# XchaoWu/ScaNeRF-Scalable-Bundle-Adjusting-Neural-Radiance-Fields-for-Large-Scale-Scene-Rendering

Hardware: NVIDIA B200
Metric: train rays/s (fwd+bwd) (higher is better)
Workload: dtype f32

## Files before the change

include/scanerf_b200.h:

```cpp
#ifndef SCANERF_B200_H
#define SCANERF_B200_H

#ifdef __cplusplus
extern "C" {
#endif

const char* snrf_last_error(void);
int snrf_version(void);
int snrf_device_sm_count(void);
int snrf_l2_fetch_granularity(int bytes);

int snrf_hash_fwd(const float* points, const float* table, const int* res, const float* corner,
                  const float* size, void* out, unsigned* idx_out, int B, int L, int T, int out_bf16,
                  void* stream);
int snrf_hash_bwd(const float* points, const float* grad_in, const float* table, const int* res,
                  const float* corner, const float* size, float* grad_points, float* grad_table,
                  int B, int L, int T, int aggregate_levels, void* stream);
void snrf_hash_set_levels_per_block(int lpb);

int snrf_field_encode_fwd(const float* rays_o, const float* rays_d, const float* z_vals, const float* points,
                          const float* box_min, const float* box_size, int mode, const float* table, const int* res,
                          float* out_lm, float* jac_lm, const unsigned char* ray_valid, int split, int N, int S, int L, int T,
                          void* stream);
int snrf_field_encode_bwd(const float* rays_o, const float* rays_d, const float* z_vals, const float* points,
// ... 63 lines not shown
                           int s_sigma, int s_tint, int s_diffuse, int s_specular,
                           const float* z_vals, const float* dists, const float* rays_d, const unsigned char* ray_valid,
                           int R, int S, int infinity, int inf_start, float* weights, float* trans, float* out,
                           float ert_eps, unsigned char* sample_live, void* stream);
int snrf_composite_bwd_ert(const float* sigma, const float* tint, const float* diffuse, const float* specular,
                           int s_sigma, int s_tint, int s_diffuse, int s_specular,
                           const float* z_vals, const float* dists, const float* rays_d, const float* trans,
                           const float* g_out, const float* g_weights, const unsigned char* ray_valid, int R, int S, int infinity,
                           int inf_start, float* g_sigma, float* g_tint, float* g_diffuse, float* g_specular,
                           int gs_sigma, int gs_tint, int gs_diffuse, int gs_specular,
                           float* grad_rays_d, const unsigned char* sample_live, void* stream);
int snrf_decoder_bwd_ert(const float* feats, const float* mask32, const float* rays_d, const float* const* params,
                         const float* grad_heads, float* grad_feats, float* grad_rays_d, float* const* grad_params,
                         int N, int S, int level_major, const unsigned char* ray_valid, const float* heads_fwd,
                         const unsigned char* sample_live, void* stream);
int snrf_field_encode_bwd_ert(const float* rays_o, const float* rays_d, const float* z_vals, const float* points,
                              const float* box_min, const float* box_size, int mode, const int* res, const float* grad_lm,
                              const float* jac_lm, float* grad_rays_o, float* grad_rays_d, float* grad_points, float* grad_table,
                              const unsigned char* ray_valid, int split, int N, int S, int L, int T,
                              const unsigned char* sample_live, void* stream);
int snrf_field_encode_bwd_adam_ert(const float* rays_o, const float* rays_d, const float* z_vals, const float* points,
                                   const float* box_min, const float* box_size, int mode, const int* res, const float* grad_lm,
                                   const float* jac_lm, float* grad_rays_o, float* grad_rays_d, float* grad_points,
                                   float* table, float* exp_avg, float* exp_avg_sq, float lr, float beta1, float beta2, float eps,
                                   int step, float* grad_scratch, long long scratch_entries, int small_levels, float* cpts_scratch,
                                   const unsigned char* ray_valid, int split, int N, int S, int L, int T,
                                   const unsigned char* sample_live, void* stream);

int snrf_joint_loss(const float* row, const unsigned char* valid_f, const unsigned char* valid_b, const float* gt,
                    float l2_weight, int R, float* loss, float* g_row, float* pred_color, int* counts_scratch, void* stream);

int snrf_umma_selftest(const float* X, const float* W, const float* G, float* Y, float* DX, float* DW,
                       float* DWo, float* YS, void* stream);

int snrf_decoder_fwd(const float* feats, const float* mask32, const float* rays_d, const float* const* params,
                     float* heads, int N, int S, int level_major, const unsigned char* ray_valid, void* stream);

void snrf_decoder_set_precision(int split);
void snrf_decoder_set_inflight(int n);
void snrf_decoder_set_fwd_fold(int on);
void snrf_decoder_set_bwd_merged(int on);
int snrf_decoder_bwd(const float* feats, const float* mask32, const float* rays_d, const float* const* params,
                     const float* grad_heads, float* grad_feats, float* grad_rays_d, float* const* grad_params,
                     int N, int S, int level_major, const unsigned char* ray_valid, const float* heads_fwd, void* stream);

int snrf_view_cost(const float* rays_o, const float* rays_d, const float* pts, const float* ks, const float* rts,
                   float* costs, int n_cam, int B, int height, int width, void* stream);
int snrf_proj2nei_fwd(const float* pts, const float* ks, const float* rts, const int* nei_views,
                      const unsigned char* nei_valid, float* nei_origin, float* nei_direction, float* grid, int B, int K,
                      void* stream);
int snrf_proj2nei_bwd(const float* pts, const float* ks, const float* rts, const int* nei_views,
                      const unsigned char* nei_valid, const float* dL_dgrid, float* grad_pts, float* grad_rts, int B, int K,
                      int n_cam, void* stream);
int snrf_grid_sample_fwd(const unsigned char* src, const float* grid, float* out, unsigned char* mask, int n_img, int B,
                         int height, int width, void* stream);
int snrf_grid_sample_bwd(const unsigned char* src, const float* grid, const float* grad_in, float* grad_grid, int n_img,
                         int B, int height, int width, void* stream);
int snrf_gauss_sample_fwd(const unsigned char* src, const float* grid, float* out, unsigned char* mask, int n_img, int B,
                          int height, int width, float sigma, float max_dis, void* stream);
int snrf_gauss_sample_bwd(const unsigned char* src, const float* grid, const float* grad_in, float* grad_grid, int n_img,
                          int B, int height, int width, float sigma, float max_dis, void* stream);
int snrf_nei_sample_fwd(const unsigned char* images, const unsigned char* occlusion, const float* grid, const int* nei_views,
                        const unsigned char* nei_valid, float* color, unsigned char* valid_out, int B, int K, int height,
                        int width, void* stream);
int snrf_nei_sample_bwd(const unsigned char* images, const float* grid, const int* nei_views, const unsigned char* nei_valid,
                        const float* grad_color, float* grad_grid, int B, int K, int height, int width, void* stream);
// ... 76 lines not shown
```

scanerf-scalable-bundle-adjusting-neural-radiance-fields-for-large-scale-scene-rendering_b200/csrc/decoder.cu:

```cuda
#include "decoder_core.cuh"

using namespace dec;

namespace {

constexpr bool kWgradDzLo = false;

template <bool SPLIT>
__global__ void __launch_bounds__(kThreadsDec, 1)
decoder_fwd_kernel(const float* __restrict__ feats, const float* __restrict__ mask32, const float* __restrict__ rays_d,
                   DecoderParams p, float* __restrict__ out, int N, int S, int num_tiles, long long level_stride,
                   const unsigned char* __restrict__ ray_valid)
{
    extern __shared__ __align__(1024) unsigned char smem_raw[];
    unsigned char* smem = (unsigned char*)(((uintptr_t)smem_raw + 1023) & ~(uintptr_t)1023);
    __shared__ uint64_t bars[2];
    __shared__ uint32_t tmem_slot;
    const int tid = threadIdx.x, warp = tid >> 5;

    stage_all_weights<SPLIT>(smem, p, mask32, tid, kThreadsDec);
    if (warp == 0) umma::tmem_alloc<512>(&tmem_slot);
    if (tid == 0) { umma::mbar_init(&bars[0], 1); umma::mbar_init(&bars[1], 1); umma::mbar_fence_init(); }
    umma::fence_async_smem();
    umma::tc_fence_before();
// ... 523 lines not shown
#pragma unroll
        for (int off = 16; off > 0; off >>= 1) {
            t2 += __shfl_xor_sync(0xffffffffu, t2, off);
            t4 += __shfl_xor_sync(0xffffffffu, t4, off);
        }
        if (lane == 0 && !first) {
            atomicAdd(gp.b2 + (j < 8 ? 8 * cg + j : 32 + 8 * cg + (j - 8)), t2 * ginv);
            atomicAdd(gp.b4 + 16 * cg + j, t4 * ginv);
        }
    }
    if (cg == 0) {
#pragma unroll
        for (int j = 0; j < 10; ++j) {
            float t = acc_small[j];
#pragma unroll
            for (int off = 16; off > 0; off >>= 1) t += __shfl_xor_sync(0xffffffffu, t, off);
            if (lane == 0 && !first) {
                float* dst = j == 0 ? gp.bs : (j < 4 ? gp.bd + (j - 1) : (j < 7 ? gp.bt + (j - 4) : gp.b5 + (j - 7)));
                atomicAdd(dst, t * ginv);
            }
        }
    }
    umma::tc_fence_before();
    __syncthreads();
    if (warp == 0) umma::tmem_free<512>(tmem);
}

namespace fold {
constexpr int oW1 = 0, oW32 = 8192, oW32l = 16384, oW3b = 24576, oW4 = 32768, oW4l = 40960, oWh2 = 49152, oWh2l = 51200,
              oW5 = 53248, oW5l = 55296, weights_end = 57344;
constexpr int oB1 = 0, oB32 = 64, oB4 = 128, nB = 192;
constexpr int off_bias = weights_end, off_mask = off_bias + nB * 4;
constexpr int off_tiles = ((off_mask + 128 + 1023) / 1024) * 1024;
constexpr int kTiles = 9;
constexpr int smem_bytes = off_tiles + kTiles * kTile + 1024;
constexpr int cDa = 0, cDb = 64, cSH = 128, gW1 = 144, gG = 192, gW3b = 256, gW4 = 272, gGhT = 336, gW5T = 352;
}

template <bool SPLIT>
__global__ void __launch_bounds__(kThreadsDec, 1)
decoder_bwd_fold_kernel(const float* __restrict__ feats, const float* __restrict__ mask32, const float* __restrict__ rays_d,
                        DecoderParams p, const float* __restrict__ grad_heads, float* __restrict__ grad_feats,
                        float* __restrict__ grad_rays_d, DecoderGrads gp, int N, int S, int num_tiles, long long level_stride,
                        const unsigned char* __restrict__ ray_valid, const unsigned* __restrict__ gmax_bits,
                        const float* __restrict__ heads_fwd, const unsigned char* __restrict__ sample_live)
{
    using namespace fold;
    extern __shared__ __align__(1024) unsigned char smem_raw[];
    unsigned char* smem = (unsigned char*)(((uintptr_t)smem_raw + 1023) & ~(uintptr_t)1023);
    unsigned char* base = smem + off_tiles;
    unsigned char *tA0 = base, *tLOb = base + kTile, *ta1 = base + 2 * kTile, *tg1 = base + 3 * kTile, *ta3 = base + 4 * kTile,
                  *tg3 = base + 5 * kTile, *ta4 = base + 6 * kTile, *tg4 = base + 7 * kTile, *tLOa = base + 8 * kTile;
    unsigned char* Tdz = tLOb;
    __shared__ uint64_t bar;
    __shared__ uint64_t bar_tail;
    __shared__ uint32_t tmem_slot;
    const int tid = threadIdx.x, warp = tid >> 5, lane = tid & 31;
    uint32_t tail_phase = 0, phase = 0;
    bool tail_pending = false;
    float gscale = 1.0f, ginv = 1.0f;
    if (kOpBf16 == 0 && gmax_bits != nullptr) {
        const int e = (int)((*gmax_bits >> 23) & 0xffu);
        if (e > 0 && e < 255) {
            int se = 253 - e;
            se = se < 1 ? 1 : (se > 253 ? 253 : se);
            gscale = __uint_as_float((uint32_t)se << 23);
            ginv = __uint_as_float((uint32_t)(254 - se) << 23);
        }
    }

    for (int i = tid; i < weights_end / 16; i += kThreadsDec) reinterpret_cast<uint4*>(smem)[i] = make_uint4(0u, 0u, 0u, 0u);
    float* s32 = reinterpret_cast<float*>(base);
    float* sh2 = s32 + 64 * 64;
    float* sW2 = sh2 + 8 * 64;
    float* sW3a = sW2 + 64 * 65;
    float* sWh = sW3a + 64 * 33;
    float* sb2 = sWh + 8 * 33;
    auto load_factors = [&]() {
        for (int i = tid; i < 64 * 64; i += kThreadsDec) sW2[(i >> 6) * 65 + (i & 63)] = w_at(p.W2, i >> 6, i & 63, 64, 64, p.flat);
        for (int i = tid; i < 64 * 32; i += kThreadsDec) sW3a[(i >> 5) * 33 + (i & 31)] = w_at(p.W3, i >> 5, i & 31, 64, 48, p.flat);
        for (int i = tid; i < 7 * 32; i += kThreadsDec) sWh[(i >> 5) * 33 + (i & 31)] = wh_at(p, i >> 5, i & 31);
        for (int i = tid; i < 64; i += kThreadsDec) sb2[i] = p.b2[i];
    };
    float* bias = reinterpret_cast<float*>(smem + off_bias);
    float* maskv = reinterpret_cast<float*>(smem + off_mask);
    load_factors();
// ... 21 lines not shown
            for (int k = 0; k < 32; ++k) v += sW3a[o * 33 + k] * sb2[32 + k];
        } else v = p.b4[i - 128];
        bias[i] = v;
    }
    for (int i = tid; i < 32; i += kThreadsDec) maskv[i] = mask32 ? mask32[i] : 1.0f;
    __syncthreads();
    stage_weight<SPLIT>(smem + oW1, smem + oW1, 0, p.W1, 64, 32, p.flat, tid, kThreadsDec);
    stage_weight<SPLIT>(smem + oW4, smem + oW4l, 0, p.W4, 64, 64, p.flat, tid, kThreadsDec);
    stage_weight<SPLIT>(smem + oW5, smem + oW5l, 0, p.W5, 3, 64, p.flat, tid, kThreadsDec);
    stage_weight<SPLIT>(smem + oW32, smem + oW32l, 0, s32, 64, 64, 0, tid, kThreadsDec);
    stage_weight<SPLIT>(smem + oWh2, smem + oWh2l, 0, sh2, 7, 64, 0, tid, kThreadsDec);
    for (int t = tid; t < 64 * 2; t += kThreadsDec) {
        const int r = t >> 1, c = t & 1;
        float hi[8], lo[8];
#pragma unroll
        for (int j = 0; j < 8; ++j) {
            const float w = w_at(p.W3, r, 32 + 8 * c + j, 64, 48, p.flat);
            hi[j] = w;
            lo[j] = w - op_round(w);
        }
        op_tile_store8(smem + oW3b, r, c, hi);
        if (SPLIT) op_tile_store8(smem + oW3b, r, 4 + c, lo);
    }
    if (warp == 0) umma::tmem_alloc<512>(&tmem_slot);
    if (tid == 0) { umma::mbar_init(&bar, 1); umma::mbar_init(&bar_tail, 1); umma::mbar_fence_init(); }
    umma::fence_async_smem();
    umma::tc_fence_before();
    __syncthreads();
    umma::tc_fence_after();

    const int row = 32 * (warp & 3) + lane, cg = warp >> 2;
    const uint32_t tmem = tmem_slot, lane_addr = (uint32_t)(32 * (warp & 3)) << 16;
    const uint32_t aA0 = umma::smem_u32(tA0), aa1 = umma::smem_u32(ta1), ag1 = umma::smem_u32(tg1), aa3 = umma::smem_u32(ta3),
                   ag3 = umma::smem_u32(tg3), aa4 = umma::smem_u32(ta4), ag4 = umma::smem_u32(tg4), aLOa = umma::smem_u32(tLOa),
                   aLOb = umma::smem_u32(tLOb), adz = aLOb;
    const uint32_t aW1 = umma::smem_u32(smem + oW1), aW32 = umma::smem_u32(smem + oW32), aW32l = umma::smem_u32(smem + oW32l),
                   aW3b = umma::smem_u32(smem + oW3b), aW4 = umma::smem_u32(smem + oW4), aW4l = umma::smem_u32(smem + oW4l),
                   aWh2 = umma::smem_u32(smem + oWh2), aWh2l = umma::smem_u32(smem + oWh2l), aW5 = umma::smem_u32(smem + oW5),
                   aW5l = umma::smem_u32(smem + oW5l);
    constexpr uint32_t idf64 = umma::idesc_f16(128, 64, 0, 0, kOpBf16, kOpBf16);
    constexpr uint32_t idg64 = umma::idesc_f16(128, 64, 0, 1, kOpBf16, kOpBf16), idg32 = umma::idesc_f16(128, 32, 0, 1, kOpBf16, kOpBf16),
                       idg16 = umma::idesc_f16(128, 16, 0, 1, kOpBf16, kOpBf16);
    constexpr uint32_t idw64 = umma::idesc_f16(64, 64, 1, 1, kOpBf16, kOpBf16), idw48 = umma::idesc_f16(64, 48, 1, 1, kOpBf16, kOpBf16),
                       idw16 = umma::idesc_f16(64, 16, 1, 1, kOpBf16, kOpBf16);
    auto dgrad = [&](int col, uint32_t dz_tile, int dz_k, uint32_t dzlo_tile, int dzlo_k, uint32_t w_hi, uint32_t w_lo, int nk,
                     uint32_t idesc, bool acc) {
        for (int k = 0; k < nk; ++k)
            umma::mma_bf16(tmem + col, umma::desc_kmajor(dz_tile, dz_k + k), umma::desc_mnmajor(w_hi, k), idesc, acc || k > 0);
        if (SPLIT) {
            for (int k = 0; k < nk; ++k)
                umma::mma_bf16(tmem + col, umma::desc_kmajor(dz_tile, dz_k + k), umma::desc_mnmajor(w_lo, k), idesc, 1);
            for (int k = 0; k < nk; ++k)
                umma::mma_bf16(tmem + col, umma::desc_kmajor(dzlo_tile, dzlo_k + k), umma::desc_mnmajor(w_hi, k), idesc, 1);
        }
    };
    auto wgrad = [&](int col, uint32_t a_tile, uint32_t b_tile_plus_off, uint32_t idesc, bool init) {
        for (int k = 0; k < 8; ++k)
            umma::mma_bf16(tmem + col, umma::desc_mnmajor(a_tile, k), umma::desc_mnmajor(b_tile_plus_off, k), idesc, (!init) || k > 0);
    };
    auto sync_operands = [&]() {
        umma::fence_async_smem();
        umma::tc_fence_before();
        __syncthreads();
        umma::tc_fence_after();
    };
    auto wait_mma = [&]() {
        umma::mbar_wait(&bar, phase);
        phase ^= 1u;
        umma::tc_fence_after();
    };
    float v[16];
    float acc_b4[16], acc_small[10];
#pragma unroll
    for (int j = 0; j < 16; ++j) acc_b4[j] = 0.0f;
#pragma unroll
    for (int j = 0; j < 10; ++j) acc_small[j] = 0.0f;
    auto gauss_epilogue = [&](int col, int boff, unsigned char* Ta, unsigned char* Tlo, unsigned char* Tg) {
        float g[16];
        umma::tmem_ld16(tmem + col + lane_addr + 16 * cg, v);
        umma::tc_wait_ld();
#pragma unroll
        for (int j = 0; j < 16; ++j) {
            const float z = v[j] + bias[boff + 16 * cg + j];
            const float a = gauss_act(z);
            v[j] = a;
            g[j] = -100.0f * z * a;
        }
#pragma unroll
        for (int q = 0; q < 2; ++q) {
            store8_act<SPLIT>(Ta, 2 * cg + q, Tlo, 2 * cg + q, row, v + 8 * q);
            umma::tile_store8_f16(Tg, row, 2 * cg + q, g + 8 * q);
        }
    };
    auto mul_inplace = [&](int col, unsigned char* Tg, unsigned char* Tlo) {
        umma::tmem_ld16(tmem + col + lane_addr + 16 * cg, v);
        umma::tc_wait_ld();
#pragma unroll
        for (int q = 0; q < 2; ++q) {
            const uint4 w4 = *reinterpret_cast<const uint4*>(Tg + umma::tile_chunk_off(row, 2 * cg + q));
            const uint32_t w[4] = {w4.x, w4.y, w4.z, w4.w};
            float o[8];
#pragma unroll
            for (int e = 0; e < 4; ++e) {
                const __half2 h2 = *reinterpret_cast<const __half2*>(&w[e]);
                o[2 * e] = v[8 * q + 2 * e] * __low2float(h2);
                o[2 * e + 1] = v[8 * q + 2 * e + 1] * __high2float(h2);
            }
            store8_act<SPLIT>(Tg, 2 * cg + q, Tlo, 2 * cg + q, row, o);
        }
    };
    const bool lead_warp = umma::warp_uniform() == 4;
    bool first = true;
    for (int tile = blockIdx.x; tile < num_tiles; tile += gridDim.x) {
        const int n = tile * kRows + row;
        const bool live = n < N && (ray_valid == nullptr || ray_valid[n / S] != 0) && (sample_live == nullptr || sample_live[n] != 0);
        if ((ray_valid != nullptr || sample_live != nullptr) && !__syncthreads_or(live)) continue;
        if (cg == 0 && live) {
            prefetch_l2(grad_heads + (size_t)n * 10);
            prefetch_l2(grad_heads + (size_t)n * 10 + 8);
            prefetch_l2(heads_fwd + (size_t)n * 10);
            prefetch_l2(heads_fwd + (size_t)n * 10 + 8);
        }
        {
            const long long nn = (long long)(tile + gridDim.x) * kRows + row;
            if (nn < N) {
                if (level_stride == 0) prefetch_l2(feats + (size_t)nn * 32 + 8 * cg);
                else {
#pragma unroll
                    for (int l = 0; l < 4; ++l) if ((row & 3) == 0) prefetch_l2(reinterpret_cast<const float2*>(feats) + nn + (size_t)(4 * cg + l) * level_stride);
                }
            }
        }
        f3 d = mk3(0.f, 0.f, 1.f);
        float dn = 1.0f;
        {
            float x[8];
#pragma unroll
            for (int j = 0; j < 8; ++j) x[j] = 0.0f;
            if (live) {
                if (level_stride == 0) {
#pragma unroll
                    for (int q = 0; q < 2; ++q) {
                        const float4 a = __ldg(reinterpret_cast<const float4*>(feats + (size_t)n * 32 + 8 * cg + 4 * q));
                        x[4 * q] = a.x; x[4 * q + 1] = a.y; x[4 * q + 2] = a.z; x[4 * q + 3] = a.w;
                    }
                } else {
                    const float2* f2 = reinterpret_cast<const float2*>(feats) + n;
#pragma unroll
                    for (int l = 0; l < 4; ++l) {
                        const float2 a = __ldg(f2 + (size_t)(4 * cg + l) * level_stride);
                        x[2 * l] = a.x; x[2 * l + 1] = a.y;
                    }
                }
                if (cg >= 2) d = ld3(rays_d + 3 * (size_t)(n / S));
#pragma unroll
                for (int j = 0; j < 8; ++j) x[j] *= maskv[8 * cg + j];
            }
            if (tail_pending) {
                umma::mbar_wait(&bar_tail, tail_phase);
                umma::tc_fence_after();
                tail_phase ^= 1u;
                tail_pending = false;
            }
            store8_act<SPLIT>(tA0, cg, tLOb, cg, row, x);
        }
        sync_operands();
        if (lead_warp && umma::elect_one()) {
            fwd_gemm<SPLIT>(tmem + cDa, aA0, 0, aLOb, 0, aW1, 0, aW1, 2, 2, idf64, false);
            umma::mma_commit(&bar);
        }
        if (cg >= 2) {
            float sh[16];
#pragma unroll
            for (int j = 0; j < 16; ++j) sh[j] = 0.0f;
            if (live) {
                dn = sqrtf(d.x * d.x + d.y * d.y + d.z * d.z);
                const float inv = 1.0f / (dn + 1e-8f);
                sh16(d.x * inv, d.y * inv, d.z * inv, sh);
            }
            store8_act<SPLIT>(tA0, 4 + (cg - 2), tA0, 6 + (cg - 2), row, sh + 8 * (cg - 2));
            if (!SPLIT) umma::tile_zero8(tA0, row, 6 + (cg - 2));
        }
        wait_mma();
        gauss_epilogue(cDa, oB1, ta1, tLOa, tg1);
        sync_operands();
        if (lead_warp && umma::elect_one()) {
            fwd_gemm<SPLIT>(tmem + cDb, aa1, 0, aLOa, 0, aW32, 0, aW32l, 0, 4, idf64, false);
            fwd_gemm<SPLIT>(tmem + cDb, aA0, 2, aA0, 3, aW3b, 0, aW3b, 2, 1, idf64, true);
            umma::mma_commit(&bar);
        }
        if (cg == 0) {
            float dzh[16], dzs[16], gh[10], hv[10];
            if (live) {
                const float2* gsrc = reinterpret_cast<const float2*>(grad_heads + (size_t)n * 10);
                const float2* hsrc = reinterpret_cast<const float2*>(heads_fwd + (size_t)n * 10);
#pragma unroll
                for (int j = 0; j < 5; ++j) {
                    const float2 t = __ldg(gsrc + j), h = __ldg(hsrc + j);
                    gh[2 * j] = t.x * gscale; gh[2 * j + 1] = t.y * gscale;
                    hv[2 * j] = h.x; hv[2 * j + 1] = h.y;
                }
            } else {
#pragma unroll
                for (int j = 0; j < 10; ++j) { gh[j] = 0.0f; hv[j] = 0.0f; }
            }
#pragma unroll
            for (int j = 0; j < 16; ++j) { dzh[j] = 0.0f; dzs[j] = 0.0f; }
            dzh[0] = gh[0] * (hv[0] > 20.0f ? 1.0f : -expm1f(-hv[0]));
#pragma unroll
            for (int j = 0; j < 3; ++j) {
                dzh[1 + j] = gh[4 + j] * hv[4 + j] * (1.0f - hv[4 + j]);
                dzh[4 + j] = gh[1 + j] * hv[1 + j] * (1.0f - hv[1 + j]);
                dzs[j] = gh[7 + j] * hv[7 + j] * (1.0f - hv[7 + j]);
            }
            store8_act<SPLIT>(Tdz, 0, Tdz, 4, row, dzh);
            store8_act<SPLIT>(Tdz, 1, Tdz, 5, row, dzh + 8);
            store8_act<SPLIT>(Tdz, 2, Tdz, 6, row, dzs);
            store8_act<SPLIT>(Tdz, 3, Tdz, 7, row, dzs + 8);
#pragma unroll
            for (int j = 0; j < 10; ++j) acc_small[j] += j < 7 ? dzh[j] : dzs[j - 7];
        }
        wait_mma();
        gauss_epilogue(cDb, oB32, ta3, tLOa, tg3);
        sync_operands();
        if (lead_warp && umma::elect_one()) {
            fwd_gemm<SPLIT>(tmem + cDa, aa3, 0, aLOa, 0, aW4, 0, aW4l, 0, 4, idf64, false);
            dgrad(cDb, adz, 1, adz, 3, aW5, aW5l, 1, idg64, false);
            umma::mma_commit(&bar);
            wgrad(gGhT, aa1, adz, idw16, first);
        }
        wait_mma();
        {
            float z4[16];
            umma::tmem_ld16(tmem + cDa + lane_addr + 16 * cg, z4);
            umma::tmem_ld16(tmem + cDb + lane_addr + 16 * cg, v);
            umma::tc_wait_ld();
#pragma unroll
            for (int j = 0; j < 16; ++j) {
                const float z = z4[j] + bias[oB4 + 16 * cg + j];
                const float a = gauss_act(z);
                z4[j] = a;
                v[j] *= -100.0f * z * a;
                acc_b4[j] += v[j];
            }
#pragma unroll
            for (int q = 0; q < 2; ++q) {
                umma::tile_store8_f16(ta4, row, 2 * cg + q, z4 + 8 * q);
                store8_act<SPLIT>(tg4, 2 * cg + q, tLOa, 2 * cg + q, row, v + 8 * q);
            }
        }
        sync_operands();
        if (lead_warp && umma::elect_one()) {
            dgrad(cDa, ag4, 0, aLOa, 0, aW4, aW4l, 4, idg64, false);
            umma::mma_commit(&bar);
            wgrad(gW4, ag4, aa3, idw64, first);
            wgrad(gW5T, aa4, adz + 32, idw16, first);
        }
        wait_mma();
        mul_inplace(cDa, tg3, tLOa);
        sync_operands();
        if (lead_warp && umma::elect_one()) {
            dgrad(cDb, ag3, 0, aLOa, 0, aW32, aW32l, 4, idg64, false);
            dgrad(cDb, adz, 0, adz, 2, aWh2, aWh2l, 1, idg64, true);
            dgrad(cSH, ag3, 0, aLOa, 0, aW3b, aW3b + 64, 4, idg16, false);
            umma::mma_commit(&bar);
            wgrad(gG, ag3, aa1, idw64, first);
            wgrad(gW3b, ag3, aA0 + 64, idw16, first);
        }
        wait_mma();
        mul_inplace(cDb, tg1, tLOa);
        sync_operands();
        if (lead_warp && umma::elect_one()) {
            dgrad(cDa, ag1, 0, aLOa, 0, aW1, aW1 + 64, 4, idg32, false);
            umma::mma_commit(&bar);
            wgrad(gW1, ag1, aA0, idw48, first);
            umma::mma_commit(&bar_tail);
        }
        if (grad_rays_d != nullptr && cg == 3) {
            float dsh[16];
            umma::tmem_ld16(tmem + cSH + lane_addr, dsh);
            umma::tc_wait_ld();
            float gx = 0.f, gy = 0.f, gz = 0.f;
            if (live) {
                const float inv = 1.0f / (dn + 1e-8f);
                const float x = d.x * inv, y = d.y * inv, z = d.z * inv;
                const float xx = x * x, yy = y * y, zz = z * z, xy = x * y, yz = y * z, xz = x * z;
                const float C1 = 0.4886025119029199f, C2a = 1.0925484305920792f, C2c = 0.31539156525252005f,
                            C2e = 0.5462742152960396f, C3a = 0.5900435899266435f, C3b = 2.890611442640554f,
                            C3c = 0.4570457994644658f, C3d = 0.3731763325901154f, C3e = 1.445305721320277f;
                float vx = 0.f, vy = 0.f, vz = 0.f;
                vy += dsh[1] * C1; vz += dsh[2] * C1; vx += dsh[3] * C1;
                vx += dsh[4] * C2a * y; vy += dsh[4] * C2a * x;
                vy += dsh[5] * -C2a * z; vz += dsh[5] * -C2a * y;
                vx += dsh[6] * C2c * -2.f * x; vy += dsh[6] * C2c * -2.f * y; vz += dsh[6] * C2c * 4.f * z;
                vx += dsh[7] * -C2a * z; vz += dsh[7] * -C2a * x;
                vx += dsh[8] * C2e * 2.f * x; vy += dsh[8] * C2e * -2.f * y;
                vx += dsh[9] * -C3a * 6.f * xy; vy += dsh[9] * -C3a * (3.f * xx - 3.f * yy);
                vx += dsh[10] * C3b * yz; vy += dsh[10] * C3b * xz; vz += dsh[10] * C3b * xy;
                vx += dsh[11] * -C3c * -2.f * xy; vy += dsh[11] * -C3c * (4.f * zz - xx - 3.f * yy); vz += dsh[11] * -C3c * 8.f * yz;
                vx += dsh[12] * C3d * -6.f * xz; vy += dsh[12] * C3d * -6.f * yz; vz += dsh[12] * C3d * (6.f * zz - 3.f * xx - 3.f * yy);
                vx += dsh[13] * -C3c * (4.f * zz - 3.f * xx - yy); vy += dsh[13] * -C3c * -2.f * xy; vz += dsh[13] * -C3c * 8.f * xz;
                vx += dsh[14] * C3e * 2.f * xz; vy += dsh[14] * C3e * -2.f * yz; vz += dsh[14] * C3e * (xx - yy);
                vx += dsh[15] * -C3a * (3.f * xx - 3.f * yy); vy += dsh[15] * -C3a * -6.f * xy;
                const float ddv = d.x * vx + d.y * vy + d.z * vz;
                const float k2 = dn > 0.f ? ddv * inv * inv / dn : 0.f;
                gx = (vx * inv - d.x * k2) * ginv; gy = (vy * inv - d.y * k2) * ginv; gz = (vz * inv - d.z * k2) * ginv;
// ... 301 lines not shown
```

scanerf-scalable-bundle-adjusting-neural-radiance-fields-for-large-scale-scene-rendering_b200/csrc/umma.cuh:

```cuda
#pragma once
#include <cuda_bf16.h>
#include <cuda_fp16.h>
#include <stdint.h>

namespace umma {

__device__ __forceinline__ uint32_t smem_u32(const void* p) { return (uint32_t)__cvta_generic_to_shared(p); }

__device__ __forceinline__ void mbar_init(uint64_t* bar, uint32_t count)
{
    asm volatile("mbarrier.init.shared::cta.b64 [%0], %1;" ::"r"(smem_u32(bar)), "r"(count));
}
__device__ __forceinline__ void mbar_fence_init() { asm volatile("fence.mbarrier_init.release.cluster;" ::: "memory"); }
__device__ __forceinline__ void mbar_wait(uint64_t* bar, uint32_t parity)
{
    asm volatile(
        "{\n"
        ".reg .pred P1;\n"
        "LAB_WAIT:\n"
        "mbarrier.try_wait.parity.shared::cta.b64 P1, [%0], %1;\n"
        "@P1 bra DONE;\n"
        "bra LAB_WAIT;\n"
        "DONE:\n"
        "}\n" ::"r"(smem_u32(bar)), "r"(parity)
// ... 34 lines not shown

__host__ __device__ constexpr uint32_t idesc_bf16(int M, int N, int a_mn_major, int b_mn_major)
{
    return (1u << 4) | (1u << 7) | (1u << 10) | ((uint32_t)a_mn_major << 15) | ((uint32_t)b_mn_major << 16) |
           ((uint32_t)(N >> 3) << 17) | ((uint32_t)(M >> 4) << 24);
}
__host__ __device__ constexpr uint32_t idesc_f16(int M, int N, int a_mn_major, int b_mn_major, int a_bf16, int b_bf16)
{
    return (1u << 4) | ((uint32_t)a_bf16 << 7) | ((uint32_t)b_bf16 << 10) | ((uint32_t)a_mn_major << 15) | ((uint32_t)b_mn_major << 16) |
           ((uint32_t)(N >> 3) << 17) | ((uint32_t)(M >> 4) << 24);
}

__device__ __forceinline__ bool elect_one()
{
    uint32_t pred;
    asm volatile(
        "{\n"
        ".reg .pred P1;\n"
        "elect.sync _|P1, 0xFFFFFFFF;\n"
        "selp.b32 %0, 1, 0, P1;\n"
        "}\n"
        : "=r"(pred));
    return pred != 0;
}
__device__ __forceinline__ int warp_uniform() { return __shfl_sync(0xffffffffu, (int)(threadIdx.x >> 5), 0); }
__device__ __forceinline__ void mma_bf16(uint32_t tmem_d, uint64_t adesc, uint64_t bdesc, uint32_t idesc, uint32_t accumulate)
{
    asm volatile(
        "{\n"
        ".reg .pred p;\n"
        "setp.ne.b32 p, %4, 0;\n"
        "tcgen05.mma.cta_group::1.kind::f16 [%0], %1, %2, %3, p;\n"
        "}\n" ::"r"(tmem_d), "l"(adesc), "l"(bdesc), "r"(idesc), "r"(accumulate)
        : "memory");
}
__device__ __forceinline__ void mma_commit(uint64_t* bar)
{
    asm volatile("tcgen05.commit.cta_group::1.mbarrier::arrive::one.shared::cluster.b64 [%0];" ::"r"(smem_u32(bar)) : "memory");
}

__device__ __forceinline__ void tmem_ld32(uint32_t taddr, float* v)
{
    uint32_t* r = reinterpret_cast<uint32_t*>(v);
    asm volatile(
        "tcgen05.ld.sync.aligned.32x32b.x32.b32 "
        "{%0, %1, %2, %3, %4, %5, %6, %7, %8, %9, %10, %11, %12, %13, %14, %15, "
        "%16, %17, %18, %19, %20, %21, %22, %23, %24, %25, %26, %27, %28, %29, %30, %31}, [%32];"
        : "=r"(r[0]), "=r"(r[1]), "=r"(r[2]), "=r"(r[3]), "=r"(r[4]), "=r"(r[5]), "=r"(r[6]), "=r"(r[7]), "=r"(r[8]),
          "=r"(r[9]), "=r"(r[10]), "=r"(r[11]), "=r"(r[12]), "=r"(r[13]), "=r"(r[14]), "=r"(r[15]), "=r"(r[16]),
          "=r"(r[17]), "=r"(r[18]), "=r"(r[19]), "=r"(r[20]), "=r"(r[21]), "=r"(r[22]), "=r"(r[23]), "=r"(r[24]),
          "=r"(r[25]), "=r"(r[26]), "=r"(r[27]), "=r"(r[28]), "=r"(r[29]), "=r"(r[30]), "=r"(r[31])
        : "r"(taddr)
        : "memory");
}
__device__ __forceinline__ void tmem_ld16(uint32_t taddr, float* v)
{
    uint32_t* r = reinterpret_cast<uint32_t*>(v);
    asm volatile(
        "tcgen05.ld.sync.aligned.32x32b.x16.b32 "
        "{%0, %1, %2, %3, %4, %5, %6, %7, %8, %9, %10, %11, %12, %13, %14, %15}, [%16];"
        : "=r"(r[0]), "=r"(r[1]), "=r"(r[2]), "=r"(r[3]), "=r"(r[4]), "=r"(r[5]), "=r"(r[6]), "=r"(r[7]), "=r"(r[8]),
          "=r"(r[9]), "=r"(r[10]), "=r"(r[11]), "=r"(r[12]), "=r"(r[13]), "=r"(r[14]), "=r"(r[15])
        : "r"(taddr)
        : "memory");
}
__device__ __forceinline__ void tmem_ld8(uint32_t taddr, float* v)
{
    uint32_t* r = reinterpret_cast<uint32_t*>(v);
    asm volatile("tcgen05.ld.sync.aligned.32x32b.x8.b32 {%0, %1, %2, %3, %4, %5, %6, %7}, [%8];"
                 : "=r"(r[0]), "=r"(r[1]), "=r"(r[2]), "=r"(r[3]), "=r"(r[4]), "=r"(r[5]), "=r"(r[6]), "=r"(r[7])
                 : "r"(taddr)
                 : "memory");
}
__device__ __forceinline__ uint32_t tmem_addr(uint32_t base, int lane, int col) { return base + ((uint32_t)lane << 16) + (uint32_t)col; }

__device__ __forceinline__ uint32_t tile_chunk_off(int row, int chunk) { return (uint32_t)row * 128u + (uint32_t)((chunk ^ (row & 7)) << 4); }

__device__ __forceinline__ uint32_t pack_bf16(float a, float b)
{
    __nv_bfloat162 h = __floats2bfloat162_rn(a, b);
    return *reinterpret_cast<uint32_t*>(&h);
}
__device__ __forceinline__ uint32_t pack_f16(float a, float b)
{
    uint32_t r;
    asm("cvt.rn.satfinite.f16x2.f32 %0, %1, %2;" : "=r"(r) : "f"(b), "f"(a));
    return r;
}
__device__ __forceinline__ void tile_store8(unsigned char* tile, int row, int chunk, const float* v)
{
    uint4 q;
    q.x = pack_bf16(v[0], v[1]); q.y = pack_bf16(v[2], v[3]); q.z = pack_bf16(v[4], v[5]); q.w = pack_bf16(v[6], v[7]);
    *reinterpret_cast<uint4*>(tile + tile_chunk_off(row, chunk)) = q;
}
__device__ __forceinline__ void tile_store8_f16(unsigned char* tile, int row, int chunk, const float* v)
{
    uint4 q;
    q.x = pack_f16(v[0], v[1]); q.y = pack_f16(v[2], v[3]); q.z = pack_f16(v[4], v[5]); q.w = pack_f16(v[6], v[7]);
    *reinterpret_cast<uint4*>(tile + tile_chunk_off(row, chunk)) = q;
}
__device__ __forceinline__ void tile_zero8(unsigned char* tile, int row, int chunk)
{
    *reinterpret_cast<uint4*>(tile + tile_chunk_off(row, chunk)) = make_uint4(0u, 0u, 0u, 0u);
}

}
```

scanerf-scalable-bundle-adjusting-neural-radiance-fields-for-large-scale-scene-rendering_b200/csrc/umma_selftest.cu:

```cuda
#include "common.cuh"
#include "umma.cuh"

namespace {

__global__ void __launch_bounds__(128, 1)
umma_selftest_kernel(const float* __restrict__ X, const float* __restrict__ W, const float* __restrict__ G,
                     float* __restrict__ Y, float* __restrict__ DX, float* __restrict__ DW,
                     float* __restrict__ DWo, float* __restrict__ YS)
{
    extern __shared__ __align__(1024) unsigned char smem_raw[];
    unsigned char* smem = (unsigned char*)(((uintptr_t)smem_raw + 1023) & ~(uintptr_t)1023);
    unsigned char* tX = smem;
    unsigned char* tG = smem + 16384;
    unsigned char* tW = smem + 32768;
    __shared__ uint64_t bar;
    __shared__ uint32_t tmem_base_slot;

    const int tid = threadIdx.x, warp = tid >> 5;
    for (int c = 0; c < 8; ++c) {
        umma::tile_store8(tX, tid, c, X + tid * 64 + c * 8);
        umma::tile_store8(tG, tid, c, G + tid * 64 + c * 8);
        if (tid < 64) umma::tile_store8(tW, tid, c, W + tid * 64 + c * 8);
    }
    if (warp == 0) umma::tmem_alloc<256>(&tmem_base_slot);
// ... 46 lines not shown
            const int m = 16 * (warp & 3) + l;
            for (int j = 0; j < 32; ++j) DW[m * 64 + 32 * h + j] = v[j];
        }
    }
    {
        float w[16];
        umma::tmem_ld16(umma::tmem_addr(tmem, lane_base, 192), w);
        umma::tc_wait_ld();
        const int l = tid & 31;
        if (l < 16) {
            const int m = 16 * (warp & 3) + l;
            for (int j = 0; j < 16; ++j) DWo[m * 16 + j] = w[j];
        }
        umma::tmem_ld16(umma::tmem_addr(tmem, lane_base, 208), w);
        umma::tc_wait_ld();
        for (int j = 0; j < 16; ++j) YS[tid * 16 + j] = w[j];
    }
    umma::tc_fence_before();
    __syncthreads();
    if (warp == 0) umma::tmem_free<256>(tmem);
}

}

SNRF_API int snrf_umma_selftest(const float* X, const float* W, const float* G, float* Y, float* DX, float* DW,
                                float* DWo, float* YS, void* stream)
{
    const int smem = 16384 * 2 + 8192 + 1024;
    cudaError_t e = cudaFuncSetAttribute(umma_selftest_kernel, cudaFuncAttributeMaxDynamicSharedMemorySize, smem);
    if (e != cudaSuccess) { snrf_set_error("snrf_umma_selftest: %s", cudaGetErrorString(e)); return (int)e; }
    umma_selftest_kernel<<<1, 128, smem, (cudaStream_t)stream>>>(X, W, G, Y, DX, DW, DWo, YS);
    SNRF_RETURN_LAUNCH("snrf_umma_selftest");
}
```

Baseline: 1.856 million.

## Feed decoder backward MMA A-operands from TMEM instead of shared memory

The fused decoder backward kernel now writes activation and gradient A-operands (hi and lo fp16 splits) into tensor memory with tcgen05.st and issues MMAs that read A from TMEM. This removes the low-part shared-memory tiles and drops one tile from the smem budget. It aims to cut shared-memory bandwidth and store traffic on the MMA operand path, at the cost of extra TMEM stores and a wait::st before each sync. Self-test and micro-benchmark probe kernels are added to check TMEM-A correctness and throughput.

Result: faster. 1.905 million, median of 6 (+2.7%).

```diff
diff --git a/include/scanerf_b200.h b/include/scanerf_b200.h
--- a/include/scanerf_b200.h
+++ b/include/scanerf_b200.h
@@ -119,6 +119,8 @@
 
 int snrf_umma_selftest(const float* X, const float* W, const float* G, float* Y, float* DX, float* DW,
                        float* DWo, float* YS, void* stream);
+int snrf_umma_selftest_tmem_a(const float* X, const float* W, const float* G, float* Y, float* DX, float* YS, void* stream);
+int snrf_umma_probe(int n, int a_tmem, int b_mn_major, int iters, int grid, long long* cycles, void* stream);
 
 int snrf_decoder_fwd(const float* feats, const float* mask32, const float* rays_d, const float* const* params,
                      float* heads, int N, int S, int level_major, const unsigned char* ray_valid, void* stream);
diff --git a/scanerf-scalable-bundle-adjusting-neural-radiance-fields-for-large-scale-scene-rendering_b200/csrc/decoder.cu b/scanerf-scalable-bundle-adjusting-neural-radiance-fields-for-large-scale-scene-rendering_b200/csrc/decoder.cu
--- a/scanerf-scalable-bundle-adjusting-neural-radiance-fields-for-large-scale-scene-rendering_b200/csrc/decoder.cu
+++ b/scanerf-scalable-bundle-adjusting-neural-radiance-fields-for-large-scale-scene-rendering_b200/csrc/decoder.cu
@@ -579,9 +579,23 @@
 constexpr int oB1 = 0, oB32 = 64, oB4 = 128, nB = 192;
 constexpr int off_bias = weights_end, off_mask = off_bias + nB * 4;
 constexpr int off_tiles = ((off_mask + 128 + 1023) / 1024) * 1024;
-constexpr int kTiles = 9;
+constexpr int kTiles = 8;
 constexpr int smem_bytes = off_tiles + kTiles * kTile + 1024;
 constexpr int cDa = 0, cDb = 64, cSH = 128, gW1 = 144, gG = 192, gW3b = 256, gW4 = 272, gGhT = 336, gW5T = 352;
+constexpr int rA = 384, rDz = 448, rSH = 480;
+
+template <bool SPLIT, int NC>
+__device__ __forceinline__ void put_operand(unsigned char* T, int row, int chunk, uint32_t hi, uint32_t lo, const float* x)
+{
+    uint32_t h[NC], l[NC];
+    umma::pack_hl_f16<NC>(x, h, l);
+#pragma unroll
+    for (int q = 0; q < NC / 4; ++q)
+        *reinterpret_cast<uint4*>(T + umma::tile_chunk_off(row, chunk + q)) = make_uint4(h[4 * q], h[4 * q + 1], h[4 * q + 2], h[4 * q + 3]);
+    if constexpr (SPLIT) umma::tmem_st_hl<NC>(hi, lo, h, l);
+    else if constexpr (NC == 4) umma::tmem_st4(hi, h);
+    else umma::tmem_st8(hi, h);
+}
 }
 
 template <bool SPLIT>
@@ -596,9 +610,9 @@
     extern __shared__ __align__(1024) unsigned char smem_raw[];
     unsigned char* smem = (unsigned char*)(((uintptr_t)smem_raw + 1023) & ~(uintptr_t)1023);
     unsigned char* base = smem + off_tiles;
-    unsigned char *tA0 = base, *tLOb = base + kTile, *ta1 = base + 2 * kTile, *tg1 = base + 3 * kTile, *ta3 = base + 4 * kTile,
-                  *tg3 = base + 5 * kTile, *ta4 = base + 6 * kTile, *tg4 = base + 7 * kTile, *tLOa = base + 8 * kTile;
-    unsigned char* Tdz = tLOb;
+    unsigned char *tA0 = base, *Tdz = base + kTile, *ta1 = base + 2 * kTile, *tg1 = base + 3 * kTile, *ta3 = base + 4 * kTile,
+                  *tg3 = base + 5 * kTile, *ta4 = base + 6 * kTile, *tg4 = base + 7 * kTile;
+    static_assert(kOpBf16 == 0, "the TMEM operands are written as fp16");
     __shared__ uint64_t bar;
     __shared__ uint64_t bar_tail;
     __shared__ uint32_t tmem_slot;
@@ -686,8 +700,7 @@
     const int row = 32 * (warp & 3) + lane, cg = warp >> 2;
     const uint32_t tmem = tmem_slot, lane_addr = (uint32_t)(32 * (warp & 3)) << 16;
     const uint32_t aA0 = umma::smem_u32(tA0), aa1 = umma::smem_u32(ta1), ag1 = umma::smem_u32(tg1), aa3 = umma::smem_u32(ta3),
-                   ag3 = umma::smem_u32(tg3), aa4 = umma::smem_u32(ta4), ag4 = umma::smem_u32(tg4), aLOa = umma::smem_u32(tLOa),
-                   aLOb = umma::smem_u32(tLOb), adz = aLOb;
+                   ag3 = umma::smem_u32(tg3), aa4 = umma::smem_u32(ta4), ag4 = umma::smem_u32(tg4), adz = umma::smem_u32(Tdz);
     const uint32_t aW1 = umma::smem_u32(smem + oW1), aW32 = umma::smem_u32(smem + oW32), aW32l = umma::smem_u32(smem + oW32l),
                    aW3b = umma::smem_u32(smem + oW3b), aW4 = umma::smem_u32(smem + oW4), aW4l = umma::smem_u32(smem + oW4l),
                    aWh2 = umma::smem_u32(smem + oWh2), aWh2l = umma::smem_u32(smem + oWh2l), aW5 = umma::smem_u32(smem + oW5),
@@ -697,15 +710,25 @@
                        idg16 = umma::idesc_f16(128, 16, 0, 1, kOpBf16, kOpBf16);
     constexpr uint32_t idw64 = umma::idesc_f16(64, 64, 1, 1, kOpBf16, kOpBf16), idw48 = umma::idesc_f16(64, 48, 1, 1, kOpBf16, kOpBf16),
                        idw16 = umma::idesc_f16(64, 16, 1, 1, kOpBf16, kOpBf16);
-    auto dgrad = [&](int col, uint32_t dz_tile, int dz_k, uint32_t dzlo_tile, int dzlo_k, uint32_t w_hi, uint32_t w_lo, int nk,
-                     uint32_t idesc, bool acc) {
+    auto fgemm = [&](int col, int a_hi, int a_lo, uint32_t w_hi, int w_hi_k, uint32_t w_lo, int w_lo_k, int nk, uint32_t idesc,
+                     bool acc) {
         for (int k = 0; k < nk; ++k)
-            umma::mma_bf16(tmem + col, umma::desc_kmajor(dz_tile, dz_k + k), umma::desc_mnmajor(w_hi, k), idesc, acc || k > 0);
+            umma::mma_f16_ta(tmem + col, tmem + a_hi + 8 * k, umma::desc_kmajor(w_hi, w_hi_k + k), idesc, acc || k > 0);
         if (SPLIT) {
             for (int k = 0; k < nk; ++k)
-                umma::mma_bf16(tmem + col, umma::desc_kmajor(dz_tile, dz_k + k), umma::desc_mnmajor(w_lo, k), idesc, 1);
+                umma::mma_f16_ta(tmem + col, tmem + a_lo + 8 * k, umma::desc_kmajor(w_hi, w_hi_k + k), idesc, 1);
             for (int k = 0; k < nk; ++k)
-                umma::mma_bf16(tmem + col, umma::desc_kmajor(dzlo_tile, dzlo_k + k), umma::desc_mnmajor(w_hi, k), idesc, 1);
+                umma::mma_f16_ta(tmem + col, tmem + a_hi + 8 * k, umma::desc_kmajor(w_lo, w_lo_k + k), idesc, 1);
+        }
+    };
+    auto dgrad = [&](int col, int dz_hi, int dz_lo, uint32_t w_hi, uint32_t w_lo, int nk, uint32_t idesc, bool acc) {
+        for (int k = 0; k < nk; ++k)
+            umma::mma_f16_ta(tmem + col, tmem + dz_hi + 8 * k, umma::desc_mnmajor(w_hi, k), idesc, acc || k > 0);
+        if (SPLIT) {
+            for (int k = 0; k < nk; ++k)
+                umma::mma_f16_ta(tmem + col, tmem + dz_hi + 8 * k, umma::desc_mnmajor(w_lo, k), idesc, 1);
+            for (int k = 0; k < nk; ++k)
+                umma::mma_f16_ta(tmem + col, tmem + dz_lo + 8 * k, umma::desc_mnmajor(w_hi, k), idesc, 1);
         }
     };
     auto wgrad = [&](int col, uint32_t a_tile, uint32_t b_tile_plus_off, uint32_t idesc, bool init) {
@@ -714,6 +737,7 @@
     };
     auto sync_operands = [&]() {
         umma::fence_async_smem();
+        umma::tc_wait_st();
         umma::tc_fence_before();
         __syncthreads();
         umma::tc_fence_after();
@@ -729,7 +753,14 @@
     for (int j = 0; j < 16; ++j) acc_b4[j] = 0.0f;
 #pragma unroll
     for (int j = 0; j < 10; ++j) acc_small[j] = 0.0f;
-    auto gauss_epilogue = [&](int col, int boff, unsigned char* Ta, unsigned char* Tlo, unsigned char* Tg) {
+    auto put8 = [&](unsigned char* T, int chunk, int hi, int lo, const float* x) {
+        put_operand<SPLIT, 4>(T, row, chunk, tmem + lane_addr + hi, tmem + lane_addr + lo, x);
+    };
+    auto put16 = [&](unsigned char* T, int chunk, int hi, int lo, const float* x) {
+        put_operand<SPLIT, 8>(T, row, chunk, tmem + lane_addr + hi, tmem + lane_addr + lo, x);
+    };
+    auto put_rA16 = [&](unsigned char* T, const float* x) { put16(T, 2 * cg, rA + 8 * cg, rA + 32 + 8 * cg, x); };
+    auto gauss_epilogue = [&](int col, int boff, unsigned char* Ta, unsigned char* Tg) {
         float g[16];
         umma::tmem_ld16(tmem + col + lane_addr + 16 * cg, v);
         umma::tc_wait_ld();
@@ -740,28 +771,26 @@
             v[j] = a;
             g[j] = -100.0f * z * a;
         }
-#pragma unroll
-        for (int q = 0; q < 2; ++q) {
-            store8_act<SPLIT>(Ta, 2 * cg + q, Tlo, 2 * cg + q, row, v + 8 * q);
-            umma::tile_store8_f16(Tg, row, 2 * cg + q, g + 8 * q);
-        }
-    };
-    auto mul_inplace = [&](int col, unsigned char* Tg, unsigned char* Tlo) {
+        put_rA16(Ta, v);
+#pragma unroll
+        for (int q = 0; q < 2; ++q) umma::tile_store8_f16(Tg, row, 2 * cg + q, g + 8 * q);
+    };
+    auto mul_inplace = [&](int col, unsigned char* Tg) {
         umma::tmem_ld16(tmem + col + lane_addr + 16 * cg, v);
         umma::tc_wait_ld();
+        float o[16];
 #pragma unroll
         for (int q = 0; q < 2; ++q) {
             const uint4 w4 = *reinterpret_cast<const uint4*>(Tg + umma::tile_chunk_off(row, 2 * cg + q));
             const uint32_t w[4] = {w4.x, w4.y, w4.z, w4.w};
-            float o[8];
 #pragma unroll
             for (int e = 0; e < 4; ++e) {
                 const __half2 h2 = *reinterpret_cast<const __half2*>(&w[e]);
-                o[2 * e] = v[8 * q + 2 * e] * __low2float(h2);
-                o[2 * e + 1] = v[8 * q + 2 * e + 1] * __high2float(h2);
-            }
-            store8_act<SPLIT>(Tg, 2 * cg + q, Tlo, 2 * cg + q, row, o);
-        }
+                o[8 * q + 2 * e] = v[8 * q + 2 * e] * __low2float(h2);
+                o[8 * q + 2 * e + 1] = v[8 * q + 2 * e + 1] * __high2float(h2);
+            }
+        }
+        put_rA16(Tg, o);
     };
     const bool lead_warp = umma::warp_uniform() == 4;
     bool first = true;
@@ -816,11 +845,11 @@
                 tail_phase ^= 1u;
                 tail_pending = false;
             }
-            store8_act<SPLIT>(tA0, cg, tLOb, cg, row, x);
+            put8(tA0, cg, rA + 4 * cg, rA + 32 + 4 * cg, x);
         }
         sync_operands();
         if (lead_warp && umma::elect_one()) {
-            fwd_gemm<SPLIT>(tmem + cDa, aA0, 0, aLOb, 0, aW1, 0, aW1, 2, 2, idf64, false);
+            fgemm(cDa, rA, rA + 32, aW1, 0, aW1, 2, 2, idf64, false);
             umma::mma_commit(&bar);
         }
         if (cg >= 2) {
@@ -832,15 +861,14 @@
                 const float inv = 1.0f / (dn + 1e-8f);
                 sh16(d.x * inv, d.y * inv, d.z * inv, sh);
             }
-            store8_act<SPLIT>(tA0, 4 + (cg - 2), tA0, 6 + (cg - 2), row, sh + 8 * (cg - 2));
-            if (!SPLIT) umma::tile_zero8(tA0, row, 6 + (cg - 2));
+            put8(tA0, 4 + (cg - 2), rSH + 4 * (cg - 2), rSH + 8 + 4 * (cg - 2), sh + 8 * (cg - 2));
         }
         wait_mma();
-        gauss_epilogue(cDa, oB1, ta1, tLOa, tg1);
+        gauss_epilogue(cDa, oB1, ta1, tg1);
         sync_operands();
         if (lead_warp && umma::elect_one()) {
-            fwd_gemm<SPLIT>(tmem + cDb, aa1, 0, aLOa, 0, aW32, 0, aW32l, 0, 4, idf64, false);
-            fwd_gemm<SPLIT>(tmem + cDb, aA0, 2, aA0, 3, aW3b, 0, aW3b, 2, 1, idf64, true);
+            fgemm(cDb, rA, rA + 32, aW32, 0, aW32l, 0, 4, idf64, false);
+            fgemm(cDb, rSH, rSH + 8, aW3b, 0, aW3b, 2, 1, idf64, true);
             umma::mma_commit(&bar);
         }
         if (cg == 0) {
@@ -867,19 +895,17 @@
                 dzh[4 + j] = gh[1 + j] * hv[1 + j] * (1.0f - hv[1 + j]);
                 dzs[j] = gh[7 + j] * hv[7 + j] * (1.0f - hv[7 + j]);
             }
-            store8_act<SPLIT>(Tdz, 0, Tdz, 4, row, dzh);
-            store8_act<SPLIT>(Tdz, 1, Tdz, 5, row, dzh + 8);
-            store8_act<SPLIT>(Tdz, 2, Tdz, 6, row, dzs);
-            store8_act<SPLIT>(Tdz, 3, Tdz, 7, row, dzs + 8);
+            put16(Tdz, 0, rDz, rDz + 16, dzh);
+            put16(Tdz, 2, rDz + 8, rDz + 24, dzs);
 #pragma unroll
             for (int j = 0; j < 10; ++j) acc_small[j] += j < 7 ? dzh[j] : dzs[j - 7];
         }
         wait_mma();
-        gauss_epilogue(cDb, oB32, ta3, tLOa, tg3);
+        gauss_epilogue(cDb, oB32, ta3, tg3);
         sync_operands();
         if (lead_warp && umma::elect_one()) {
-            fwd_gemm<SPLIT>(tmem + cDa, aa3, 0, aLOa, 0, aW4, 0, aW4l, 0, 4, idf64, false);
-            dgrad(cDb, adz, 1, adz, 3, aW5, aW5l, 1, idg64, false);
+            fgemm(cDa, rA, rA + 32, aW4, 0, aW4l, 0, 4, idf64, false);
+            dgrad(cDb, rDz + 8, rDz + 24, aW5, aW5l, 1, idg64, false);
             umma::mma_commit(&bar);
             wgrad(gGhT, aa1, adz, idw16, first);
         }
@@ -898,34 +924,32 @@
                 acc_b4[j] += v[j];
             }
 #pragma unroll
-            for (int q = 0; q < 2; ++q) {
-                umma::tile_store8_f16(ta4, row, 2 * cg + q, z4 + 8 * q);
-                store8_act<SPLIT>(tg4, 2 * cg + q, tLOa, 2 * cg + q, row, v + 8 * q);
-            }
+            for (int q = 0; q < 2; ++q) umma::tile_store8_f16(ta4, row, 2 * cg + q, z4 + 8 * q);
+            put_rA16(tg4, v);
         }
         sync_operands();
         if (lead_warp && umma::elect_one()) {
-            dgrad(cDa, ag4, 0, aLOa, 0, aW4, aW4l, 4, idg64, false);
+            dgrad(cDa, rA, rA + 32, aW4, aW4l, 4, idg64, false);
             umma::mma_commit(&bar);
             wgrad(gW4, ag4, aa3, idw64, first);
             wgrad(gW5T, aa4, adz + 32, idw16, first);
         }
         wait_mma();
-        mul_inplace(cDa, tg3, tLOa);
+        mul_inplace(cDa, tg3);
         sync_operands();
         if (lead_warp && umma::elect_one()) {
-            dgrad(cDb, ag3, 0, aLOa, 0, aW32, aW32l, 4, idg64, false);
-            dgrad(cDb, adz, 0, adz, 2, aWh2, aWh2l, 1, idg64, true);
-            dgrad(cSH, ag3, 0, aLOa, 0, aW3b, aW3b + 64, 4, idg16, false);
+            dgrad(cDb, rA, rA + 32, aW32, aW32l, 4, idg64, false);
+            dgrad(cDb, rDz, rDz + 16, aWh2, aWh2l, 1, idg64, true);
+            dgrad(cSH, rA, rA + 32, aW3b, aW3b + 64, 4, idg16, false);
             umma::mma_commit(&bar);
             wgrad(gG, ag3, aa1, idw64, first);
             wgrad(gW3b, ag3, aA0 + 64, idw16, first);
         }
         wait_mma();
-        mul_inplace(cDb, tg1, tLOa);
+        mul_inplace(cDb, tg1);
         sync_operands();
         if (lead_warp && umma::elect_one()) {
-            dgrad(cDa, ag1, 0, aLOa, 0, aW1, aW1 + 64, 4, idg32, false);
+            dgrad(cDa, rA, rA + 32, aW1, aW1 + 64, 4, idg32, false);
             umma::mma_commit(&bar);
             wgrad(gW1, ag1, aA0, idw48, first);
             umma::mma_commit(&bar_tail);
diff --git a/scanerf-scalable-bundle-adjusting-neural-radiance-fields-for-large-scale-scene-rendering_b200/csrc/umma.cuh b/scanerf-scalable-bundle-adjusting-neural-radiance-fields-for-large-scale-scene-rendering_b200/csrc/umma.cuh
--- a/scanerf-scalable-bundle-adjusting-neural-radiance-fields-for-large-scale-scene-rendering_b200/csrc/umma.cuh
+++ b/scanerf-scalable-bundle-adjusting-neural-radiance-fields-for-large-scale-scene-rendering_b200/csrc/umma.cuh
@@ -90,6 +90,16 @@
         "setp.ne.b32 p, %4, 0;\n"
         "tcgen05.mma.cta_group::1.kind::f16 [%0], %1, %2, %3, p;\n"
         "}\n" ::"r"(tmem_d), "l"(adesc), "l"(bdesc), "r"(idesc), "r"(accumulate)
+        : "memory");
+}
+__device__ __forceinline__ void mma_f16_ta(uint32_t tmem_d, uint32_t tmem_a, uint64_t bdesc, uint32_t idesc, uint32_t accumulate)
+{
+    asm volatile(
+        "{\n"
+        ".reg .pred p;\n"
+        "setp.ne.b32 p, %4, 0;\n"
+        "tcgen05.mma.cta_group::1.kind::f16 [%0], [%1], %2, %3, p;\n"
+        "}\n" ::"r"(tmem_d), "r"(tmem_a), "l"(bdesc), "r"(idesc), "r"(accumulate)
         : "memory");
 }
 __device__ __forceinline__ void mma_commit(uint64_t* bar)
@@ -130,6 +140,20 @@
                  : "r"(taddr)
                  : "memory");
 }
+__device__ __forceinline__ void tmem_st4(uint32_t taddr, const uint32_t* r)
+{
+    asm volatile("tcgen05.st.sync.aligned.32x32b.x4.b32 [%0], {%1, %2, %3, %4};" ::"r"(taddr), "r"(r[0]), "r"(r[1]), "r"(r[2]),
+                 "r"(r[3])
+                 : "memory");
+}
+__device__ __forceinline__ void tmem_st8(uint32_t taddr, const uint32_t* r)
+{
+    asm volatile("tcgen05.st.sync.aligned.32x32b.x8.b32 [%0], {%1, %2, %3, %4, %5, %6, %7, %8};" ::"r"(taddr), "r"(r[0]), "r"(r[1]),
+                 "r"(r[2]), "r"(r[3]), "r"(r[4]), "r"(r[5]), "r"(r[6]), "r"(r[7])
+                 : "memory");
+}
+__device__ __forceinline__ void tc_wait_st() { asm volatile("tcgen05.wait::st.sync.aligned;" ::: "memory"); }
+
 __device__ __forceinline__ uint32_t tmem_addr(uint32_t base, int lane, int col) { return base + ((uint32_t)lane << 16) + (uint32_t)col; }
 
 __device__ __forceinline__ uint32_t tile_chunk_off(int row, int chunk) { return (uint32_t)row * 128u + (uint32_t)((chunk ^ (row & 7)) << 4); }
@@ -145,6 +169,23 @@
     asm("cvt.rn.satfinite.f16x2.f32 %0, %1, %2;" : "=r"(r) : "f"(b), "f"(a));
     return r;
 }
+template <int NC>
+__device__ __forceinline__ void pack_hl_f16(const float* v, uint32_t* h, uint32_t* l)
+{
+#pragma unroll
+    for (int i = 0; i < NC; ++i) {
+        h[i] = pack_f16(v[2 * i], v[2 * i + 1]);
+        const float2 f = __half22float2(*reinterpret_cast<const __half2*>(&h[i]));
+        l[i] = pack_f16(v[2 * i] - f.x, v[2 * i + 1] - f.y);
+    }
+}
+template <int NC>
+__device__ __forceinline__ void tmem_st_hl(uint32_t hi, uint32_t lo, const uint32_t* h, const uint32_t* l)
+{
+    static_assert(NC == 4 || NC == 8, "x4 or x8");
+    if constexpr (NC == 4) { tmem_st4(hi, h); tmem_st4(lo, l); }
+    else { tmem_st8(hi, h); tmem_st8(lo, l); }
+}
 __device__ __forceinline__ void tile_store8(unsigned char* tile, int row, int chunk, const float* v)
 {
     uint4 q;
diff --git a/scanerf-scalable-bundle-adjusting-neural-radiance-fields-for-large-scale-scene-rendering_b200/csrc/umma_selftest.cu b/scanerf-scalable-bundle-adjusting-neural-radiance-fields-for-large-scale-scene-rendering_b200/csrc/umma_selftest.cu
--- a/scanerf-scalable-bundle-adjusting-neural-radiance-fields-for-large-scale-scene-rendering_b200/csrc/umma_selftest.cu
+++ b/scanerf-scalable-bundle-adjusting-neural-radiance-fields-for-large-scale-scene-rendering_b200/csrc/umma_selftest.cu
@@ -102,3 +102,139 @@
     umma_selftest_kernel<<<1, 128, smem, (cudaStream_t)stream>>>(X, W, G, Y, DX, DW, DWo, YS);
     SNRF_RETURN_LAUNCH("snrf_umma_selftest");
 }
+
+namespace {
+
+__global__ void __launch_bounds__(128, 1)
+umma_selftest_tmem_a_kernel(const float* __restrict__ X, const float* __restrict__ W, const float* __restrict__ G,
+                            float* __restrict__ Y, float* __restrict__ DX, float* __restrict__ YS)
+{
+    extern __shared__ __align__(1024) unsigned char smem_raw[];
+    unsigned char* tW = (unsigned char*)(((uintptr_t)smem_raw + 1023) & ~(uintptr_t)1023);
+    __shared__ uint64_t bar;
+    __shared__ uint32_t tmem_base_slot;
+    constexpr int cY = 0, cDX = 64, cYS = 128, aX = 256, aG = 320;
+
+    const int tid = threadIdx.x, warp = tid >> 5;
+    if (tid < 64)
+        for (int c = 0; c < 8; ++c) umma::tile_store8_f16(tW, tid, c, W + tid * 64 + c * 8);
+    if (warp == 0) umma::tmem_alloc<512>(&tmem_base_slot);
+    if (tid == 0) { umma::mbar_init(&bar, 1); umma::mbar_fence_init(); }
+    umma::fence_async_smem();
+    umma::tc_fence_before();
+    __syncthreads();
+    umma::tc_fence_after();
+    const uint32_t tmem = tmem_base_slot, lane_addr = (uint32_t)(32 * warp) << 16;
+    for (int q = 0; q < 4; ++q) {
+        uint32_t h[8], l[8];
+        umma::pack_hl_f16<8>(X + tid * 64 + 16 * q, h, l);
+        umma::tmem_st_hl<8>(tmem + lane_addr + aX + 8 * q, tmem + lane_addr + aX + 32 + 8 * q, h, l);
+        umma::pack_hl_f16<8>(G + tid * 64 + 16 * q, h, l);
+        umma::tmem_st_hl<8>(tmem + lane_addr + aG + 8 * q, tmem + lane_addr + aG + 32 + 8 * q, h, l);
+    }
+    umma::tc_wait_st();
+    umma::tc_fence_before();
+    __syncthreads();
+    umma::tc_fence_after();
+
+    if (warp == 0 && umma::elect_one()) {
+        const uint32_t bW = umma::smem_u32(tW);
+        const uint32_t id_y = umma::idesc_f16(128, 64, 0, 0, 0, 0), id_dx = umma::idesc_f16(128, 64, 0, 1, 0, 0),
+                       id_ys = umma::idesc_f16(128, 16, 0, 0, 0, 0);
+        for (int k = 0; k < 4; ++k) umma::mma_f16_ta(tmem + cY, tmem + aX + 8 * k, umma::desc_kmajor(bW, k), id_y, k > 0);
+        for (int k = 0; k < 4; ++k) umma::mma_f16_ta(tmem + cY, tmem + aX + 32 + 8 * k, umma::desc_kmajor(bW, k), id_y, 1);
+        for (int k = 0; k < 4; ++k) umma::mma_f16_ta(tmem + cDX, tmem + aG + 8 * k, umma::desc_mnmajor(bW, k), id_dx, k > 0);
+        for (int k = 0; k < 4; ++k) umma::mma_f16_ta(tmem + cDX, tmem + aG + 32 + 8 * k, umma::desc_mnmajor(bW, k), id_dx, 1);
+        for (int k = 0; k < 2; ++k) umma::mma_f16_ta(tmem + cYS, tmem + aX + 16 + 8 * k, umma::desc_kmajor(bW, k), id_ys, k > 0);
+        umma::mma_commit(&bar);
+    }
+    umma::mbar_wait(&bar, 0);
+    umma::tc_fence_after();
+
+    float v[32];
+    for (int h = 0; h < 2; ++h) {
+        umma::tmem_ld32(tmem + lane_addr + cY + 32 * h, v);
+        umma::tc_wait_ld();
+        for (int j = 0; j < 32; ++j) Y[tid * 64 + 32 * h + j] = v[j];
+        umma::tmem_ld32(tmem + lane_addr + cDX + 32 * h, v);
+        umma::tc_wait_ld();
+        for (int j = 0; j < 32; ++j) DX[tid * 64 + 32 * h + j] = v[j];
+    }
+    umma::tmem_ld16(tmem + lane_addr + cYS, v);
+    umma::tc_wait_ld();
+    for (int j = 0; j < 16; ++j) YS[tid * 16 + j] = v[j];
+    umma::tc_fence_before();
+    __syncthreads();
+    if (warp == 0) umma::tmem_free<512>(tmem);
+}
+
+__global__ void __launch_bounds__(128, 1)
+umma_probe_kernel(int n, int a_tmem, int b_mn_major, int iters, long long* __restrict__ cycles)
+{
+    extern __shared__ __align__(1024) unsigned char smem_raw[];
+    unsigned char* tA = (unsigned char*)(((uintptr_t)smem_raw + 1023) & ~(uintptr_t)1023);
+    unsigned char* tB = tA + 16384;
+    __shared__ uint64_t bar;
+    __shared__ uint32_t tmem_base_slot;
+    const int tid = threadIdx.x, warp = tid >> 5;
+    for (int i = tid; i < 24576 / 16; i += 128) reinterpret_cast<uint4*>(tA)[i] = make_uint4(0u, 0u, 0u, 0u);
+    if (warp == 0) umma::tmem_alloc<256>(&tmem_base_slot);
+    if (tid == 0) { umma::mbar_init(&bar, 1); umma::mbar_fence_init(); }
+    umma::fence_async_smem();
+    umma::tc_fence_before();
+    __syncthreads();
+    umma::tc_fence_after();
+    const uint32_t tmem = tmem_base_slot;
+    {
+        const uint32_t z[8] = {0u, 0u, 0u, 0u, 0u, 0u, 0u, 0u};
+        for (int c = 0; c < 32; c += 8) umma::tmem_st8(tmem + ((uint32_t)(32 * warp) << 16) + 128 + c, z);
+        umma::tc_wait_st();
+    }
+    umma::tc_fence_before();
+    __syncthreads();
+    umma::tc_fence_after();
+    const bool issuer = warp == 0 && umma::elect_one();
+    long long t0 = 0;
+    if (issuer) {
+        const uint32_t aA = umma::smem_u32(tA), aB = umma::smem_u32(tB);
+        const uint32_t idesc = umma::idesc_f16(128, n, 0, b_mn_major, 0, 0);
+        t0 = clock64();
+        for (int it = 0; it < iters; ++it) {
+#pragma unroll
+            for (int k = 0; k < 4; ++k) {
+                const uint64_t bd = b_mn_major ? umma::desc_mnmajor(aB, k) : umma::desc_kmajor(aB, k);
+                if (a_tmem) umma::mma_f16_ta(tmem, tmem + 128 + 8 * k, bd, idesc, 1);
+                else umma::mma_bf16(tmem, umma::desc_kmajor(aA, k), bd, idesc, 1);
+            }
+        }
+        umma::mma_commit(&bar);
+    }
+    umma::mbar_wait(&bar, 0);
+    if (issuer) cycles[blockIdx.x] = clock64() - t0;
+    umma::tc_fence_after();
+    umma::tc_fence_before();
+    __syncthreads();
+    if (warp == 0) umma::tmem_free<256>(tmem);
+}
+
+}
+
+SNRF_API int snrf_umma_selftest_tmem_a(const float* X, const float* W, const float* G, float* Y, float* DX, float* YS, void* stream)
+{
+    const int smem = 8192 + 1024;
+    umma_selftest_tmem_a_kernel<<<1, 128, smem, (cudaStream_t)stream>>>(X, W, G, Y, DX, YS);
+    SNRF_RETURN_LAUNCH("snrf_umma_selftest_tmem_a");
+}
+
+SNRF_API int snrf_umma_probe(int n, int a_tmem, int b_mn_major, int iters, int grid, long long* cycles, void* stream)
+{
+    if ((n != 16 && n != 32 && n != 64) || iters < 1 || grid < 1) {
+        snrf_set_error("snrf_umma_probe: n must be 16, 32 or 64, iters and grid positive (got %d, %d, %d)", n, iters, grid);
+        return 1;
+    }
+    const int smem = 128 * 1024 + 1024;
+    cudaError_t e = cudaFuncSetAttribute(umma_probe_kernel, cudaFuncAttributeMaxDynamicSharedMemorySize, smem);
+    if (e != cudaSuccess) { snrf_set_error("snrf_umma_probe: %s", cudaGetErrorString(e)); return (int)e; }
+    umma_probe_kernel<<<grid, 128, smem, (cudaStream_t)stream>>>(n, a_tmem, b_mn_major, iters, cycles);
+    SNRF_RETURN_LAUNCH("snrf_umma_probe");
+}
```
